# PolyU-IOR/HPR-LP-C

Hardware: AMD Instinct MI355X
Metric: HPR iterations/sec (FP64) (higher is better)
Workload: dtype f64

## Files before the change

### hpr-lp-c_amd/csrc/abi.cpp

```cpp
#include <algorithm>
#include <cmath>
#include <cstdlib>
#include <cstring>
#include <memory>
#include <mutex>
#include <iomanip>
#include <iostream>

#include "hprlp_amd.h"
#include "env.h"
#include "dist.h"
#include "presolve.h"
#include "reorder.h"
#include "solver.h"
#include "version.h"

using namespace hprlp;

struct hprlp_solver {
    Solver s;
    Comm *comm = nullptr;
    Comm *xcomm = nullptr;
    bool sharded = false;
    ~hprlp_solver() {}
// ... 1169 lines not shown
    auto one = [](const char *name, const DeviceMatrix &M) {
        const TiledDev &t = M.view.tiled;
        std::string d = std::string(name) + ": ";
        if (!t.valid) {
            d += "stream kernel (k_spmv_fused, " + std::to_string(M.view.nblk) + " row blocks, " + std::to_string(M.view.nlong) + " split rows)";
            d += no_tiled_note(M.outcome.why);
            return d;
        }
        d += t.n_pieces > 0 ? "tiled, piece form (k_tiled_part + k_tiled_finish, " + std::to_string(t.n_pieces) + " pieces)"
             : t.rem_cap == kPbRemCap ? "tiled, all-remainder form (k_pb_fused, grid " + std::to_string(t.grid) + ")"
                                      : "tiled, fused (k_tiled_fused, grid " + std::to_string(t.grid) + ")";
        d += ", " + std::to_string(t.nsb) + " super-blocks, " + std::to_string(M.tiled.n_steps) + " steps";
        if (t.R != kTileRows || t.T != kTileCols) d += " (" + std::to_string(t.R) + " rows, tiles of " + std::to_string(t.T) + " columns)";
        const double all = static_cast<double>(M.tiled.dense_entries) + static_cast<double>(M.tiled.n_rem);
        if (all > 0) d += ", " + std::to_string(static_cast<int>(100.0 * M.tiled.dense_entries / all + 0.5)) + " % of the entries in staged tiles";
        if (t.f_rk) d += ", source-side run tables";
        if (t.f_work) d += ", pre-pass work list of " + std::to_string(t.n_work) + " workgroups for " + std::to_string(t.n_groups) + " source groups";
        if (t.side_nblk > 0) d += ", long rows aside (" + std::to_string(t.side_nblk) + " blocks through the stream kernel)";
        return d;
    };
    std::string d = one("A", s.A) + "; " + one("A^T", s.AT);
    if (s.use_small && !s.comm) d += "; normal iterations in the single-workgroup kernel (k_small_iterations)";
    if (!s.perm_r.empty()) d += "; locality ordering applied at set-up";
    if (!s.env_at_setup.empty()) d += "; switches: " + s.env_at_setup;
    if (!s.env_ignored_at_setup.empty()) d += "; ignored without HPRLP_TEST_HOOKS=1: " + s.env_ignored_at_setup;
    std::snprintf(buf, static_cast<size_t>(cap), "%s", d.c_str());
    return static_cast<int>(d.size());
    GUARD_END(-1)
}

extern "C" int hprlp_form_select(const hprlp_form_facts *facts, const hprlp_form_hooks *hooks, hprlp_form_decision *out) {
// ... 12 lines not shown
extern "C" int hprlp_solver_form_facts(hprlp_solver *h, int which, hprlp_form_facts out[2]) {
    GUARD_BEGIN
    if (!h || !out || which < 0 || which > 1) throw std::runtime_error("null solver / buffer, or no such matrix");
    h->s.finish_tiling();
    const DeviceMatrix &M = which ? h->s.AT : h->s.A;
    out[0] = M.facts;
    out[1] = M.facts_pb;
    return M.passes;
    GUARD_END(-1)
}

extern "C" int hprlp_tiled_host_check(int m, int n, const int *rowptr, const int *col, int R, int T, double min_dense, long out[6]) {
    try {
        if (m <= 0 || n <= 0 || !rowptr || !col || !out) throw std::runtime_error("bad arguments");
        tiled_host_check(m, n, rowptr, col, R, T, min_dense, out);
        return 0;
    } catch (const std::exception &e) {
        set_last_error(e.what());
        return -1;
    }
}

extern "C" int hprlp_env_switches(char *buf, int cap) {
    int count = 0;
    const EnvEntry *t = env_table(&count);
    std::string d;
    for (int i = 0; i < count; ++i) d += std::string(t[i].name) + "\t" + (t[i].kind == EnvKind::Integrator ? "integrator" : "hook") + "\t" + t[i].what + "\n";
    if (buf && cap > 0) std::snprintf(buf, static_cast<size_t>(cap), "%s", d.c_str());
    return static_cast<int>(d.size());
}
// ... 68 lines not shown
```

### hpr-lp-c_amd/csrc/env.cpp

```cpp
#include "env.h"

#include <cstdlib>
#include <cstring>
#include <stdexcept>

namespace hprlp {

static const EnvEntry kTable[] = {
    {"HPRLP_TEST_HOOKS", EnvKind::Integrator, "1: honour the test hooks below (tests/conftest.py and the tools/ scripts set it)"},
    {"HPRLP_TIMING", EnvKind::Integrator, "wall time of the set-up and solve phases on stderr"},
    {"HPRLP_NO_GRAPH", EnvKind::Integrator, "launch normal iterations eagerly instead of replaying hipGraphs (fall-back)"},
    {"HPRLP_NO_TILED", EnvKind::Integrator, "never build the column-tiled matrix copies: stream kernel everywhere (fall-back)"},
    {"HPRLP_NO_REORDER", EnvKind::Integrator, "no set-up time locality ordering of a large matrix"},
    {"HPRLP_NO_ALLOC_CACHE", EnvKind::Integrator, "do not keep freed device blocks for the next solver of the process"},
    {"HPRLP_DIST_TRANSPORT", EnvKind::Integrator, "shm: hprlp_dist_unique_id names a shared-memory segment (host-staged group of processes on one node) instead of RCCL ids"},
    {"HPRLP_NO_WARM_MODEL", EnvKind::Integrator, "the model constructors do NOT start the HIP runtime / device context / code objects (for a process that forks workers after building its models: a HIP context does not survive fork); the first solve pays for them as in the reference"},
    {"HPRLP_DIST_EXCHANGE", EnvKind::Hook, "sparse | allgather: force the multi-GPU exchange form (same value on every rank)"},
    {"HPRLP_NO_OVERLAP", EnvKind::Integrator, "multi-GPU: shards unsplit, exchange in line on the solver stream"},
    {"HPRLP_DIST_TIMEOUT_S", EnvKind::Integrator, "seconds a rank of the shared-memory transport waits for its peers before it fails (default 120)"},
    {"HPRLP_BATCH_CHUNK", EnvKind::Hook, "solve_batched with 64 or more problems: chunk width of the panels (default 64; narrower chunks map one chunk to each XCD -- measured slower, profiles/r03_tiled_decomposition.md section 6b)"},
    {"HPRLP_BATCH_GRID", EnvKind::Hook, "solve_batched: cap on the row blocks of the normal half-step kernels (read at every call; a small cap makes every workgroup's row loop wrap)"},
    {"HPRLP_BATCH_LAMBDA", EnvKind::Hook, "solve_batched: the batch's lambda_max from the caller (strtod; hand it over as a C99 hex float to keep every bit) instead of 1.01 x the power iteration's estimate (read at every call)"},
    {"HPRLP_COPY_PAUSE_US", EnvKind::Hook, "piece size and pause of the threaded copies of set-up (64 MB, 100 us)"},
    {"HPRLP_COPY_PIECE_MB", EnvKind::Hook, "piece size and pause of the threaded copies of set-up (64 MB, 100 us)"},
    {"HPRLP_DEVICE_TRANSPOSE_MIN", EnvKind::Hook, "build Aᵀ on the host / nonzero threshold of the device transpose (default 4 M)"},
    {"HPRLP_DIST_SELFTEST_FAIL", EnvKind::Hook, "tests only: the set-up self-test of the neighbour exchange reports a failure once (exercises the fall-back to the all-gather)"},
    {"HPRLP_DTON_MAX", EnvKind::Hook, "presolve: cap of the doubleton stage"},
    {"HPRLP_DTON_TRACE", EnvKind::Hook, "presolve: trace the doubleton stage on stderr"},
    {"HPRLP_GEN_FAR", EnvKind::Hook, "benchmark generator: share of a row's entries that fall anywhere (default 0.05)"},
    {"HPRLP_HOST_POWER_START", EnvKind::Hook, "power iteration's start vector made on the host also above 1e6 rows (default there: on the device)"},
    {"HPRLP_HOST_TILING", EnvKind::Hook, "build the tiled copies with the host builder (background threads, default min(16, cores)) instead of on the device"},
    {"HPRLP_HOST_TRANSPOSE", EnvKind::Hook, "build Aᵀ on the host / nonzero threshold of the device transpose (default 4 M)"},
    {"HPRLP_NO_BOUND_CODES", EnvKind::Hook, "the x-half always reads l[j] and u[j], the y-half AL[i] and AU[i] (default: one code byte per column / row says which of them is not a constant; an equality row reads one value)"},
    {"HPRLP_NO_FAR_PUSH", EnvKind::Hook, "always run the remainder pre-pass (k_far_products) instead of the hand-off from the producing half-step's epilogue"},
    {"HPRLP_NO_FAR_WORK", EnvKind::Hook, "the remainder pre-pass with one workgroup per source group also where one group holds several times the mean (default: a work list cuts heavy groups into chunks, tiled.h f_work)"},
    {"HPRLP_NO_PB_LONG_ROWS", EnvKind::Hook, "a matrix kept off the tiled forms for its long rows keeps the stream kernel also where its columns are not popular (default: all-remainder form, Solver::pb_fallback_wanted)"},
    {"HPRLP_NO_FUSED_NORMS", EnvKind::Hook, "the Ruiz row norms by their own passes instead of as a by-product of the preceding scaling pass (same bits)"},
    {"HPRLP_NO_LONG_SIDE", EnvKind::Hook, "a matrix with rows over 1024 entries keeps the stream kernel instead of being tiled with those rows kept aside"},
    {"HPRLP_NO_PB_FALLBACK", EnvKind::Hook, "unstructured large matrices keep the stream kernel instead of the tiled form without dense-tile requirement"},
    {"HPRLP_NO_PB_KERNEL", EnvKind::Hook, "run an all-remainder copy through k_tiled_fused's remainder steps instead of k_pb_fused (A/B)"},
    {"HPRLP_NO_REM2", EnvKind::Hook, "tiled build: no second remainder level"},
    {"HPRLP_NO_SETUP_OVERLAP", EnvKind::Hook, "set-up of a large model in line: no helper threads / copy streams for the value upload, the row blocks, A^T's row pointers and the model vectors (same bits either way)"},
    {"HPRLP_NO_SLAB_CUTS", EnvKind::Hook, "dense rows of a large matrix are not cut at the XCD eighths of the gathered vector (stream kernel)"},
    {"HPRLP_NO_SMALL", EnvKind::Hook, "do not use the single-workgroup kernel for Netlib-scale LPs"},
    {"HPRLP_NO_SMALL_POWER", EnvKind::Hook, "Netlib-scale LPs: power iteration by the regular kernels with the host test every 10th iteration (default: one launch of the single-workgroup kernel)"},
    {"HPRLP_NO_TILED_CR", EnvKind::Hook, "Curtis-Reid passes through the stream kernel also for matrices with a tiled copy (default: tiled kernel on a second value array of -log|a|)"},
    {"HPRLP_NT", EnvKind::Hook, "force default / nontemporal loads of the matrix in the stream kernel"},
    {"HPRLP_OVERLAP_COMM_FIRST", EnvKind::Hook, "tests only: with the in-process rank group, use RCCL's launch order (exchange enqueued before the local SpMV)"},
    {"HPRLP_PB_MIN_COLS", EnvKind::Hook, "gathered-vector length from which an unstructured matrix takes the all-remainder form (default 800 k columns, the crossover measured with k_pb_fused)"},
// ... 64 lines not shown
```

### hpr-lp-c_amd/csrc/kernels.h

```cpp
#pragma once

#include <hip/hip_runtime.h>

#include "tiled.h"

namespace hprlp {

constexpr int kWave = 64;
constexpr int kWavesPerBlock = 4;
constexpr int kThreads = kWave * kWavesPerBlock;
constexpr int kStreamW = 512;
constexpr int kStreamRows = 64;
constexpr int kLongRow = 64;
constexpr int kSplitRow = 4096;
constexpr int kNumScalars = 32;

enum Slot : int {
    S_CX = 0,
    S_YOBJ_Y = 1,
    S_XZ = 2,
    S_RD2 = 3,
    S_RP2 = 4,
    S_ADX_DY = 5,
    S_DY2 = 6,
// ... 47 lines not shown
};

struct Ctrl {
    double sigma, lam_sigma, inv_lam_sigma, inv_sigma;
    int kx, ky;
    int pad0, pad1;
};

struct FarPush {
    const int *gptr = nullptr;
    const double *val = nullptr;
    const int *pos = nullptr;
    const uint16_t *lcol = nullptr;
    double *P = nullptr;
    const int *rptr = nullptr, *rk = nullptr, *rp = nullptr;
};

struct XHalfArgs {
    const double *y_full;
    double *x, *x_hat;
    const double *l, *u, *c, *last_x;
    double *x_bar, *z_bar, *x_temp;
    Ctrl *ctrl;
    double *partials;
    int stride;
    FarPush push;
    bool far_ready = false;
    const unsigned char *lu_code = nullptr;
    int x_mode = 0;
};
// ... 17 lines not shown
void launch_row_codes(int m, const double *AL, const double *AU, unsigned char *code, hipStream_t s);

struct FinalizeItem {
    const double *partials;
    int count;
    int slot;
    int max = 0;
};
struct FinalizeArgs {
    FinalizeItem item[8];
    int n;
};

bool launch_x_half(const CsrDev &AT, const XHalfArgs &a, bool check, hipStream_t s);
bool launch_y_half(const CsrDev &A, const YHalfArgs &a, bool check, hipStream_t s);
FarPush far_push_of(const CsrDev &consumer);
void launch_x_half_base(const CsrDev &AT_remote, const XHalfArgs &a, const double *base, hipStream_t s);
void launch_y_half_base(const CsrDev &A_remote, const YHalfArgs &a, const double *base, hipStream_t s);

void launch_resid_d(const CsrDev &AT, const double *ybar_full, const double *c, const double *z_bar,
                    const double *col_norm, double *partials, hipStream_t s);
void launch_resid_p(const CsrDev &A, const double *xbar_full, const double *xtemp_full, const double *AL,
                    const double *AU, const double *row_norm, const double *y_temp, bool with_gap,
                    double *partials, int stride, hipStream_t s);
void launch_gap(const CsrDev &A, const double *xtemp_full, const double *y_temp, double *partials, hipStream_t s);
bool launch_spmv_push(const CsrDev &M, const double *v_full, double *out, const FarPush &push, hipStream_t s);
void launch_spmv_plain(const CsrDev &M, const double *v_full, double *out, const double *q, bool with_dots,
                       double *partials, int stride, hipStream_t s, bool far_ready = false);

void launch_finalize(const FinalizeArgs &f, double *scalars, hipStream_t s);

// ... 115 lines not shown
```

### hpr-lp-c_amd/csrc/kernels.hip

```cpp
#include "kernels.h"

#include <algorithm>
#include <vector>
#include <cmath>
#include <type_traits>

namespace hprlp {

__device__ __forceinline__ double wave_sum(double v) {
#pragma unroll
    for (int off = 32; off > 0; off >>= 1) v += __shfl_xor(v, off, kWave);
    return v;
}

__device__ __forceinline__ double wave_max(double v) {
#pragma unroll
    for (int off = 32; off > 0; off >>= 1) v = fmax(v, __shfl_xor(v, off, kWave));
    return v;
}

template <int NACC, int NW, int NMAX = 0>
__device__ __forceinline__ void block_store_partials_in(double (&acc)[NACC], double *partials, int stride, double (*red)[NACC > 0 ? NACC : 1]) {
    const int wave = threadIdx.x >> 6, lane = threadIdx.x & 63;
#pragma unroll
// ... 580 lines not shown
        for (int u = 0; u < U; ++u)
            if (k + u * NT < pe) f.P[ps[u]] = prd[u];
    }
}

__device__ __forceinline__ int run_position(const int *tab_k, const int *tab_p, int nr, int k) {
    int lo = 0, hi = nr - 1;
    while (lo < hi) {
        const int mid = (lo + hi + 1) >> 1;
        if (tab_k[mid] <= k) lo = mid;
        else hi = mid - 1;
    }
    return tab_p[lo] + (k - tab_k[lo]);
}

__device__ __forceinline__ void push_products_runs(const FarPush &f, const double *vals, int *tab, int g, int pb, int pe, int tid) {
    constexpr int NT = kTileThreads, U = 4;
    if (pb >= pe) return;
    const int r0 = f.rptr[g], nr = f.rptr[g + 1] - r0;
    int *tab_k = tab, *tab_p = tab + kPbRunTabCap;
    double a4[U];
    uint16_t c4[U];
    auto load_batch = [&](int k0) {
#pragma unroll
        for (int u = 0; u < U; ++u) {
            const int z = min(k0 + u * NT, pe - 1);
            a4[u] = __builtin_nontemporal_load(f.val + z);
            c4[u] = __builtin_nontemporal_load(f.lcol + z);
        }
    };
    int k = pb + tid;
    load_batch(k);
    for (int i = tid; i < nr; i += NT) {
        tab_k[i] = f.rk[r0 + i];
        tab_p[i] = f.rp[r0 + i];
// ... 6 lines not shown
        double prd[U];
        int pc[U];
#pragma unroll
        for (int u = 0; u < U; ++u) {
            prd[u] = a4[u] * vals[c4[u]];
            pc[u] = ps[u];
        }
        const int kn = k + U * NT;
        if (kn < pe) load_batch(kn);
#pragma unroll
        for (int u = 0; u < U; ++u)
            if (k + u * NT < pe) f.P[pc[u]] = prd[u];
        if (kn < pe) {
#pragma unroll
            for (int u = 0; u < U; ++u) ps[u] = run_position(tab_k, tab_p, nr, min(kn + u * NT, pe - 1));
        }
    }
}

template <class Epi, bool REP, bool PUSH = false, bool NARROW = false>
__global__ void __launch_bounds__(kTileThreads, 4) k_tiled_fused(CsrDev A, Epi epi) {
    static_assert(Epi::NV == 1, "the tiled kernel stages one gathered vector");
    constexpr int NT = kTileThreads, RMAX = kTileRows, T = kTileCols;
    constexpr int NACC = Epi::NACC;
    __shared__ double acc[RMAX];
    __shared__ __attribute__((aligned(16))) double ytile[T];
    const TiledDev &t = A.tiled;
    const int tid = threadIdx.x;
    const int R = t.R;
    const int per = t.per, slots = gridDim.x / 8;
// ... 2 lines not shown
#pragma unroll
    for (int i = 0; i < (NACC > 0 ? NACC : 1); ++i) racc[i] = 0.0;
    epi.begin();
    int wg_round = 0;
    const bool wg_stamp = t.wgtimes && tid == 0 && (t.wg_filter == 0 || (PUSH && NACC == 0));
    if (wg_stamp) t.wgtimes[blockIdx.x * 8] = wall_clock64();
    for (int q = slot; q < per; q += slots) {
        const int sb = (blockIdx.x % 8) * per + q;
        if (sb >= t.nsb) break;
        const double *__restrict__ vec = epi.gv[0];
        lds_barrier();
        const int ncols = A.cols;
        for (int i = tid; i < R; i += NT) acc[i] = 0.0;
        const int s0 = t.sb_ptr[sb], smid = t.sb_mid[sb], s1 = t.sb_ptr[sb + 1];
        if (s0 < smid) tiled_sweep<HPRLP_SWEEP_ED, HPRLP_SWEEP_TD, REP, false, LogTerm<Epi>::value, NARROW ? kTileColsNarrow : kTileCols>(t, s0, smid - s0, t.steps[s0].rot, smid - s0, vec, ncols, acc, ytile, tid);
        remainder_steps<kTileRemK>(t, smid, s1, acc, ytile, ytile + kTileRemCap, tid);
        lds_barrier();
        const int r0 = sb * R;
        const int nr = min(R, A.rows - r0);
        int pb = 0, pe = 0;
        if constexpr (PUSH) {
            pb = epi.push.gptr[sb];
            pe = epi.push.gptr[sb + 1];
        }
        epilogue_rows<Epi, PUSH>(epi, acc, racc, r0, nr, tid);
        if constexpr (PUSH) {
            lds_barrier();
            push_products(epi.push, acc, pb, pe, tid);
        }
        if (wg_stamp && ++wg_round <= 5) t.wgtimes[blockIdx.x * 8 + wg_round] = wall_clock64();
    }
    if (wg_stamp) {
        t.wgtimes[blockIdx.x * 8 + 7] = wall_clock64();
        const unsigned hw = __builtin_amdgcn_s_getreg((31 << 11) | 4), xcc = __builtin_amdgcn_s_getreg((31 << 11) | 20);
        t.wgtimes[blockIdx.x * 8 + 6] = (static_cast<unsigned long long>(xcc & 0xfu) << 32) | hw;
    }
    if constexpr (NACC > 0) {
        __syncthreads();
        block_store_partials_in<NACC, kTileThreads / kWave, MaxAccs<Epi>::value>(racc, epi.partials, epi.stride, reinterpret_cast<double(*)[NACC]>(ytile));
    }
}

template <class Epi, bool PUSH = false>
// ... 256 lines not shown
        const int kn = k + U * kFarThreads;
        if (kn < e) load_batch(kn);
#pragma unroll
        for (int u = 0; u < U; ++u)
            if (k + u * kFarThreads < e) t.P[pc[u]] = pr[u];
        if (kn < e) {
#pragma unroll
            for (int u = 0; u < U; ++u) ps[u] = run_position(tab_k, tab_p, nr, min(kn + u * kFarThreads, e - 1));
        }
    }
}

template <bool LOGTERM>
static void launch_far_products(const TiledDev &t, const double *vec, int ncols, hipStream_t s) {
    const dim3 grid(((t.f_work ? t.n_work : t.n_groups) + 7) / 8 * 8);
    if (t.f_rk && t.G <= kPbRowsMax) hipLaunchKernelGGL(k_far_products_runs<LOGTERM>, grid, dim3(kFarThreads), 0, s, t, vec, ncols);
    else hipLaunchKernelGGL(k_far_products<LOGTERM>, grid, dim3(kFarThreads), 0, s, t, vec, ncols);
}


template <bool CHECK, bool STREAMED = false>
struct XEpi {
    static constexpr int NV = 1;
    static constexpr int NACC = CHECK ? 3 : 0;
    const double *gv[1];
    double *x, *x_hat;
    const double *l, *u, *c, *last_x;
    double *x_bar, *z_bar, *x_temp;
    Ctrl *ctrl;
    double *partials;
    int stride;
// ... 424 lines not shown
    }
    if constexpr (Publishes<Epi>::value) {
        if (e.push.gptr) {
            if (narrow) hipLaunchKernelGGL((k_tiled_fused<Epi, false, true, true>), dim3(M.tiled.grid), dim3(kTileThreads), 0, s, M, e);
            else if (M.tiled.repeats) hipLaunchKernelGGL((k_tiled_fused<Epi, true, true>), dim3(M.tiled.grid), dim3(kTileThreads), 0, s, M, e);
            else hipLaunchKernelGGL((k_tiled_fused<Epi, false, true>), dim3(M.tiled.grid), dim3(kTileThreads), 0, s, M, e);
            return true;
        }
    }
    if (narrow) hipLaunchKernelGGL((k_tiled_fused<Epi, false, false, true>), dim3(M.tiled.grid), dim3(kTileThreads), 0, s, M, e);
    else if (M.tiled.repeats) hipLaunchKernelGGL((k_tiled_fused<Epi, true>), dim3(M.tiled.grid), dim3(kTileThreads), 0, s, M, e);
    else hipLaunchKernelGGL((k_tiled_fused<Epi, false>), dim3(M.tiled.grid), dim3(kTileThreads), 0, s, M, e);
    return false;
}

FarPush far_push_of(const CsrDev &consumer) {
    FarPush f;
    if (consumer.tiled.valid && consumer.tiled.n_groups > 0) {
        f.gptr = consumer.tiled.f_gptr;
        f.val = consumer.tiled.f_val;
        f.pos = consumer.tiled.f_pos;
        f.lcol = consumer.tiled.f_lcol;
        f.P = consumer.tiled.P;
        if (consumer.tiled.f_rk) {
            f.rptr = consumer.tiled.f_rptr;
            f.rk = consumer.tiled.f_rk;
            f.rp = consumer.tiled.f_rp;
        }
    }
    return f;
}

bool launch_x_half(const CsrDev &AT, const XHalfArgs &a, bool check, hipStream_t s) {
    if (check) {
        XEpi<true> e{{a.y_full}, a.x, a.x_hat, a.l, a.u, a.c, a.last_x, a.x_bar, a.z_bar, a.x_temp, a.ctrl, a.partials, a.stride, 0, 0, 0, a.push, a.lu_code};
        return launch_fused(AT, e, s, a.far_ready);
    }
    if (AT.tiled.valid) {
        XEpi<false, true> e{{a.y_full}, a.x, a.x_hat, a.l, a.u, a.c, a.last_x, nullptr, nullptr, nullptr, a.ctrl, nullptr, 0, 0, 0, 0, a.push, a.lu_code, a.x_mode};
// ... 1006 lines not shown
```

### hpr-lp-c_amd/csrc/solver.cpp

```cpp
#include "solver.h"
#include "env.h"

#include <algorithm>
#include <cmath>
#include <cstdio>
#include <cstdlib>
#include <cstring>
#include <functional>
#include <iomanip>
#include <iostream>
#include <limits>
#include <thread>

#include "dist.h"
#include "reorder.h"

namespace hprlp {

constexpr int kMaxGraphIters = 64;
constexpr int kDeviceStartRows = 1000000;
constexpr int kPowerBlockKey = -10;

struct RowCuts {
    std::vector<int> rows;
// ... 1297 lines not shown
    HIP_CHECK(hipMemsetAsync(gsm.p, 0, sizeof(double) * m_pad, stream));
    HIP_CHECK(hipMemsetAsync(gsn.p, 0, sizeof(double) * n_pad, stream));
    HIP_CHECK(hipStreamSynchronize(stream));
    power_time = time_since(t0);
    return lambda;
}

void Solver::set_sigma_lambda(double sigma_, double lambda_, bool reset_k) {
    sigma = sigma_;
    lambda_max = lambda_;
    launch_set_ctrl(ctrl.p, sigma, lambda_max, reset_k ? 1 : 0, stream);
}

void Solver::read_hooks() {
    hook_no_far_push = env_get("HPRLP_NO_FAR_PUSH") && env_get("HPRLP_NO_FAR_PUSH")[0] == '1';
    hook_no_bound_codes = env_get("HPRLP_NO_BOUND_CODES") != nullptr;
    hook_store_x = env_get("HPRLP_STORE_X") != nullptr;
}

void Solver::refresh_bound_codes() {
    if (hook_no_bound_codes) return;
    if (n_loc > 0) {
        if (lu_code.n != static_cast<size_t>(n_loc)) lu_code.alloc(static_cast<size_t>(n_loc));
        launch_bound_codes(n_loc, l.p, u.p, lu_code.p, stream);
    }
    if (m_loc > 0) {
        if (row_code.n != static_cast<size_t>(m_loc)) row_code.alloc(static_cast<size_t>(m_loc));
        launch_row_codes(m_loc, AL.p, AU.p, row_code.p, stream);
    }
}
// ... 53 lines not shown
    finish_tiling();
    HIP_CHECK(hipStreamSynchronize(stream));
    ensure_comm_stream();
    ovAT.reset(new SplitShard);
    split_shard(AT, row_off, row_off + m_loc, ovAT.get(), stream);
    ovA.reset(new SplitShard);
    split_shard(A, col_off, col_off + n_loc, ovA.get(), stream);
    HIP_CHECK(hipDeviceSynchronize());
    overlap_ready = true;
}

FarPush Solver::push_into(const DeviceMatrix &consumer, const DeviceMatrix &producer) const {
    const TiledDev &pt = producer.view.tiled;
    if (hook_no_far_push || comm || !pt.valid || pt.n_pieces > 0) return FarPush{};
    if (consumer.view.tiled.valid && consumer.view.tiled.G != pt.R) return FarPush{};
    return far_push_of(consumer.view);
}

int Solver::x_mode_of(int i, int count) const {
    if (hook_store_x || overlap_enabled || !AT.view.tiled.valid) return 0;
    return (i > 0 ? kXRebuild : 0) | (i + 1 < count ? kXNoStore : 0);
}

void Solver::launch_normal_pair(bool more_follow, hipEvent_t *ev, int x_mode) {
    XHalfArgs xa{gy.p, x.p, x_hat, l.p, u.p, c.p, last_x.p, nullptr, nullptr, nullptr, ctrl.p, nullptr, 0};
    xa.lu_code = lu_code.p;
    xa.x_mode = x_mode;
    YHalfArgs ya{gxh.p, y, AL.p, AU.p, last_y.p, nullptr, nullptr, nullptr, ctrl.p, nullptr, 0};
    ya.row_code = row_code.p;
    if (ev) HIP_CHECK(hipEventRecord(ev[0], stream));
    if (!overlap_enabled) {
// ... 542 lines not shown
```

### hpr-lp-c_amd/csrc/solver.h

```cpp
#pragma once

#include <string>
#include <vector>

#include <functional>
#include <future>
#include <map>
#include <memory>

#include "common.h"
#include "env.h"
#include "dist.h"
#include "kernels.h"
#include "hpr_rules.h"
#include "form_select.h"

namespace hprlp {

HPRLP_batched_results solve_batched_impl(const LP_info_cpu *model, int batch_size, const HPRLP_FLOAT *C, const HPRLP_FLOAT *AL,
                                         const HPRLP_FLOAT *AU, const HPRLP_FLOAT *l, const HPRLP_FLOAT *u,
                                         const HPRLP_FLOAT *obj_constants, const HPRLP_parameters *param, const Detection *det,
                                         std::vector<Certificate> *certs, const HPRLP_FLOAT *X0 = nullptr,
                                         const HPRLP_FLOAT *Y0 = nullptr);
HPRLP_batched_results make_batched_error(const char *status, int m, int n, int B);
// ... 145 lines not shown
    void collect_solution(HPRLP_results *out);
    double reduce_sum_sq(const double *v, int n_local);
    void verify_exchange();
    void gather(double *gbuf, bool is_m) { gather_on(gbuf, is_m, stream); }
    void gather_on(double *gbuf, bool is_m, hipStream_t s);

    struct SplitShard {
        DeviceMatrix loc, rem;
        DBuf<double> part;
    };
    std::unique_ptr<SplitShard> ovA, ovAT;
    hipStream_t comm_stream = nullptr;
    hipEvent_t ev_ready = nullptr, ev_done_x = nullptr, ev_done_y = nullptr;
    std::string env_at_setup, env_ignored_at_setup;
    bool hook_no_far_push = false, hook_no_bound_codes = false, hook_store_x = false;
    void read_hooks();
    bool overlap_enabled = false, overlap_ready = false, y_exchange_pending = false;
    bool overlap_spmv_first = false;
    void prepare_overlap();
    void ensure_comm_stream();
    void allreduce_scalars();
    void finish_tiling();

    void launch_normal_pair(bool more_follow = false, hipEvent_t *ev = nullptr, int x_mode = 0);
    int x_mode_of(int i, int count) const;

   private:
    void alloc_work();
    hipGraphExec_t graph_for(int len);
};
// ... 3 lines not shown
```

### hpr-lp-c_amd/csrc/tiled.cpp

```cpp
#include "tiled.h"
#include "env.h"

#include <algorithm>
#include <cstdlib>
#include <cstring>
#include <string>
#include <thread>
#include <type_traits>

namespace hprlp {

namespace {

struct Local {
    std::vector<int> sb_steps, sb_mid;
    std::vector<TileStep> steps;
    std::vector<char> step_is_rem;
    std::vector<uint32_t> tidx;
    std::vector<int> tperm, rcol, rperm;
    std::vector<uint16_t> rrow;
    long dense = 0, pad = 0;
};

void build_range(int rows, int cols, const int *rp, const int *ci, int sb0, int sb1, Local *L, int R, int T, int rem_cap) {
// ... 266 lines not shown
                if (row_of(k) != sb * R + rrow[e]) throw std::runtime_error("tiled check: a remainder entry in the wrong super-block / row");
            }
        }
    }
    for (long k = 0; k < nnz; ++k)
        if (!seen[k]) throw std::runtime_error("tiled check: an entry is missing");
    if (most_run > kTileLayers * ((static_cast<long>(R) * kTileChunk + kTileStepCap - 1) / kTileStepCap + 1)) throw std::runtime_error("tiled check: too many steps for one tile");
    out[0] = static_cast<long>(h.n_tile);
    out[1] = static_cast<long>(h.n_rem);
    out[2] = static_cast<long>(h.steps.size());
    out[3] = pads;
    out[4] = most_run;
    out[5] = static_cast<long>(1e6 * static_cast<double>(h.dense_entries) / static_cast<double>(nnz));
}

void DeviceTiled::upload(const TiledHost &h, int R, int T, int rem_cap) {
    n_tile = static_cast<long>(h.n_tile);
    n_rem = static_cast<long>(h.n_rem);
    n_steps = static_cast<int>(h.steps.size());
    const int nsb = static_cast<int>(h.sb_mid.size());
    sb_ptr.alloc(h.sb_ptr.size()); sb_ptr.upload(h.sb_ptr.data(), h.sb_ptr.size());
    sb_mid.alloc(h.sb_mid.size()); sb_mid.upload(h.sb_mid.data(), h.sb_mid.size());
    steps.alloc(h.steps.size()); steps.upload(h.steps.data(), h.steps.size());
    tidx.alloc_zero(h.n_tile + 8);
    tperm.alloc(h.n_tile + 8);
    tval.alloc_zero(h.n_tile + 8);
    rcol.alloc_zero(h.n_rem + 8);
    rperm.alloc(h.n_rem + 8);
    rrow.alloc_zero(h.n_rem + 8);
    size_t to = 0, ro = 0;
// ... 77 lines not shown
```

### hpr-lp-c_amd/csrc/tiled.h

```cpp
#pragma once

#include <hip/hip_runtime.h>

#include <cstdint>
#include <vector>

#include "common.h"

namespace hprlp {

constexpr int kTileThreads = 512;
constexpr int kTileRows = 8192;
constexpr int kTileCols = 2048;
constexpr int kTileColsNarrow = 1024;
constexpr int kTileChunk = 4;
constexpr int kTileStepCap = kTileThreads * kTileChunk;
constexpr int kTileRemK = 4;
constexpr int kTileRemCap = (kTileThreads - 4) * kTileRemK;
constexpr int kTileRemRun = 16;
#ifndef HPRLP_PB_REM_K
#define HPRLP_PB_REM_K 8
#endif
constexpr int kPbRemK = HPRLP_PB_REM_K;
constexpr int kPbRemCap = kTileThreads * kPbRemK;
constexpr int kPbRowsMax = 4096;
constexpr int kPbRunTabCap = 3072;
constexpr int kTileMaxRow = 1024;
constexpr int kTileDenseMin = 256;
static_assert(kTileRemCap % kTileRemK == 0 && kTileRemCap + (kTileThreads / 64) * 3 / 2 <= kTileCols, "tile buffer too small for the remainder scratch");
constexpr int kTileRowBits = 13;
constexpr int kTileRowsMin = 1024;
static_assert((1 << kTileRowBits) == kTileRows && kTileCols <= (1 << (24 - kTileRowBits)) && kTileChunk == 4,
              "entry codes are 24 bits: 13 of local row, 11 of local column, four per chunk");
inline uint32_t tile_code(int lcol, int row) { return (static_cast<uint32_t>(lcol) << kTileRowBits) | static_cast<uint32_t>(row); }

struct PackLayout {
    int n1 = 0, n2 = 0, n3 = 0, n4 = 0;
    int u3 = 0, u2 = 0, r1 = 0, c2 = 0;
    __host__ __device__ void set(int a1, int a2, int a3, int a4) {
        n1 = a1; n2 = a2; n3 = a3; n4 = a4;
        u3 = n1 < n3 ? n1 : n3;
// ... 78 lines not shown
    const int *sb_mid = nullptr;
    const TileStep *steps = nullptr;
    const double *tval = nullptr;
    const uint32_t *tidx3 = nullptr;
    double *P = nullptr;
    const uint32_t *rq = nullptr;
    int n_groups = 0;
    const int *f_gptr = nullptr;
    const double *f_val = nullptr;
    const int *f_pos = nullptr;
    const uint16_t *f_lcol = nullptr;
    const int *f_rptr = nullptr;
    const int *f_rk = nullptr;
    const int *f_rp = nullptr;
    int f_maxruns = 0;
    const int4 *f_work = nullptr;
    int n_work = 0;
};

struct TiledHost {
    std::vector<int> sb_ptr, sb_mid;
    std::vector<TileStep> steps;
    struct Piece {
        std::vector<uint32_t> tidx;
        std::vector<int> tperm;
        std::vector<int> rcol, rperm;
        std::vector<uint16_t> rrow;
    };
    std::vector<Piece> pieces;
    size_t n_tile = 0, n_rem = 0;
    long dense_entries = 0;
    long padding = 0;
};

bool build_tiled(int rows, int cols, const int *rowptr, const int *col, TiledHost *out, int min_rows,
                 double min_dense_fraction, int R = kTileRows, int T = kTileCols, int rem_cap = kTileRemCap);

void tiled_host_check(int rows, int cols, const int *rp, const int *ci, int R, int T, double min_dense, long out[6]);

void compact_without_rows(long nnz, int rows, const int *rp_dev, const int *rp_c_dev, const int *col_dev, int *col_c, int *map_c, hipStream_t s);

struct DeviceTiled {
    DBuf<int> sb_ptr, sb_mid, tperm, rperm, rcol;
    DBuf<TileStep> steps;
    DBuf<uint32_t> tidx;
    DBuf<uint32_t> tidx3;
    DBuf<uint16_t> rrow;
    DBuf<double> tval;
    DBuf<double> P, f_val;
    DBuf<uint32_t> rq;
    DBuf<int> f_gptr, f_pos, f_perm;
    DBuf<int> f_rptr, f_rk, f_rp;
    DBuf<int4> f_work;
// ... 33 lines not shown
```

### hpr-lp-c_amd/csrc/tiled_build.hip

```cpp
#include <algorithm>
#include <functional>
#include <cstdlib>
#include <hipcub/hipcub.hpp>

#include <vector>

#include "common.h"
#include "env.h"
#include "kernels.h"
#include "tiled.h"

namespace hprlp {

namespace {

constexpr int K = kTileChunk;
constexpr int kRowBits = kTileRowBits;

__device__ __forceinline__ int row_of_entry(const int *__restrict__ rowptr, int rows, int k) {
    int lo = 0, hi = rows;
    while (hi - lo > 1) {
        const int mid = lo + ((hi - lo) >> 1);
        if (rowptr[mid] <= k) lo = mid;
        else hi = mid;
// ... 789 lines not shown
                if (e <= b) continue;
                const long parts = (e - b + cap - 1) / cap, per = (e - b + parts - 1) / parts;
                for (long q = b; q < e; q += per) wl.push_back(make_int4(g, static_cast<int>(q), static_cast<int>(std::min(e, q + per)), 0));
            }
            f_work.alloc(wl.size());
            f_work.upload(wl.data(), wl.size());
            view.f_work = f_work.p;
            view.n_work = static_cast<int>(wl.size());
            if (env_get("HPRLP_TIMING"))
                std::fprintf(stderr, "[timing]   pre-pass work list: %d workgroups for %d source groups (heaviest group %d entries, chunks of at most %ld)\n",
                             view.n_work, ngroups, heaviest, cap);
        }
    }
    view.f_rptr = view.f_rk = view.f_rp = nullptr;
    view.f_maxruns = 0;
    if (view.rem_cap == kPbRemCap) {
        DBuf<int> flag(static_cast<size_t>(n)), excl(static_cast<size_t>(n));
        hipLaunchKernelGGL(k_far_run_flags, dim3(grid_for(n)), dim3(kThreads), 0, s, n, kout.p, f_pos.p, flag.p);
        size_t bytes = 0;
        HIP_CHECK(hipcub::DeviceScan::ExclusiveSum(nullptr, bytes, flag.p, excl.p, n, s));
        {
            DBuf<char> tmp(bytes + 16);
            HIP_CHECK(hipcub::DeviceScan::ExclusiveSum(tmp.p, bytes, flag.p, excl.p, n, s));
            HIP_CHECK(hipStreamSynchronize(s));
        }
        int last_excl = 0, last_flag = 0;
        HIP_CHECK(hipMemcpy(&last_excl, excl.p + (n - 1), sizeof(int), hipMemcpyDeviceToHost));
        HIP_CHECK(hipMemcpy(&last_flag, flag.p + (n - 1), sizeof(int), hipMemcpyDeviceToHost));
        const int nruns = last_excl + last_flag;
        f_rk.alloc(static_cast<size_t>(nruns) + 8);
        f_rp.alloc(static_cast<size_t>(nruns) + 8);
        f_rptr.alloc(static_cast<size_t>(ngroups) + 1);
        DBuf<int> mx;
        mx.alloc_zero(1);
        hipLaunchKernelGGL(k_far_run_fill, dim3(grid_for(n)), dim3(kThreads), 0, s, n, flag.p, excl.p, f_pos.p, f_rk.p, f_rp.p);
        hipLaunchKernelGGL(k_far_rptr, dim3(grid_for(ngroups + 1)), dim3(kThreads), 0, s, ngroups, n, nruns, f_gptr.p, excl.p, f_rptr.p, mx.p);
        int h_mx = 0;
        HIP_CHECK(hipMemcpyAsync(&h_mx, mx.p, sizeof(int), hipMemcpyDeviceToHost, s));
        HIP_CHECK(hipStreamSynchronize(s));
        if (h_mx > 0 && h_mx <= kPbRunTabCap && static_cast<long>(n) >= 48L * nruns) {
            view.f_rptr = f_rptr.p;
            view.f_rk = f_rk.p;
            view.f_rp = f_rp.p;
            view.f_maxruns = h_mx;
        }
        if (env_get("HPRLP_TIMING"))
            std::fprintf(stderr, "[timing]   source-side run tables: %d runs of %d entries (%.1f per run), most in one group %d%s\n", nruns, n,
                         static_cast<double>(n) / std::max(nruns, 1), h_mx, view.f_rk ? "" : " -- not used (too many for the producers' LDS table)");
    }
    rcol.release(); rrow.release(); rperm.release();
    view.P = P.p;
    view.rq = rq.p;
    view.n_groups = ngroups;
    view.f_gptr = f_gptr.p;
    view.f_val = f_val.p;
    view.f_pos = f_pos.p;
    view.f_lcol = f_lcol.p;
}

// ... 166 lines not shown
```

### include/hprlp_amd.h

```cpp
#ifndef HPRLP_AMD_H
#define HPRLP_AMD_H

#include "HPRLP.h"

#ifdef __cplusplus
extern "C" {
#endif

typedef struct hprlp_solver hprlp_solver;

typedef struct hprlp_trace_row {
    int iter, restart_flag;
    double err_Rp, err_Rd, primal_obj, dual_obj, gap, kkt, sigma, current_gap, lambda_max;
} hprlp_trace_row;

const char *hprlp_last_error(void);
const char *hprlp_backend(void);
int hprlp_warmup(int device);
int hprlp_warmup_seconds(double out[4]);

void hprlp_release_device_cache(void);
int hprlp_alloc_cache_selftest(void);

hprlp_solver *hprlp_solver_create(const LP_info_cpu *model, const HPRLP_parameters *param);
// ... 111 lines not shown
                                                   hprlp_local_group *group);

typedef struct hprlp_presolve hprlp_presolve;
hprlp_presolve *hprlp_presolve_run(const LP_info_cpu *model);
const LP_info_cpu *hprlp_presolve_reduced(const hprlp_presolve *p);
int hprlp_presolve_stats(const hprlp_presolve *p, int out[16]);
int hprlp_presolve_postsolve(const hprlp_presolve *p, const double *xr, const double *yr, const double *zr, double *x,
                             double *y, double *z);
int hprlp_presolve_forward(const hprlp_presolve *p, const double *x, const double *y, double *xr, double *yr);
void hprlp_presolve_free(hprlp_presolve *p);
int hprlp_original_kkt(const LP_info_cpu *model, const double *x, const double *y, const double *z, double out[5]);

int hprlp_locality_ordering(int m, int n, const int *rowptr, const int *col, int *row_new2old, int *col_new2old, double out[6]);
int hprlp_row_block_plan(int m, int n, const int *rowptr, const int *col, int with_cuts, long out[6]);
int hprlp_tiled_host_check(int m, int n, const int *rowptr, const int *col, int R, int T, double min_dense, long out[6]);

typedef struct hprlp_form_built {
    long ok;
    long n_pieces, dense_entries, n_rem;
    double rem_top_share;
} hprlp_form_built;
typedef struct hprlp_form_facts {
    long rows, cols, nnz, longest_row;
    double long_row_share;
    double line_density;
    double xcd_gather_bytes;
    long sb_rows, slots;
    double min_dense_override;
    long sharded;
    long heaviest_block;
// ... 35 lines not shown
```

Baseline: 748.7.

## Use run tables and early-issued loads in the tiled fused kernel's hand-off

Extends the source-side run tables, previously built only for the all-remainder form, to the tiled fused kernel's far-product hand-off, so it can compute write positions from a small LDS run table instead of reading f_pos per entry. It also issues the first trip of hand-off loads (values, local columns, run entries) before the epilogue so their latency overlaps epilogue work. The cost is more registers held across the epilogue, a reused LDS scratch area, and an extra table build for all matrices. A hook picks the mode, and a host reference builder is added for testing.

Measured after the change: 748.5 (median of 3 runs). About the same (-0.0%).

```diff
diff --git a/hpr-lp-c_amd/csrc/abi.cpp b/hpr-lp-c_amd/csrc/abi.cpp
--- a/hpr-lp-c_amd/csrc/abi.cpp
+++ b/hpr-lp-c_amd/csrc/abi.cpp
@@ -1207,7 +1207,9 @@
         if (t.R != kTileRows || t.T != kTileCols) d += " (" + std::to_string(t.R) + " rows, tiles of " + std::to_string(t.T) + " columns)";
         const double all = static_cast<double>(M.tiled.dense_entries) + static_cast<double>(M.tiled.n_rem);
         if (all > 0) d += ", " + std::to_string(static_cast<int>(100.0 * M.tiled.dense_entries / all + 0.5)) + " % of the entries in staged tiles";
-        if (t.f_rk) d += ", source-side run tables";
+        if (t.f_rk) d += t.rem_cap == kPbRemCap ? ", source-side run tables" : ", hand-off positions from run tables";
+        else if (t.n_groups > 0 && t.rem_cap != kPbRemCap && t.f_maxruns > kTileRunTabCap)
+            d += ", hand-off positions kept in f_pos (" + std::to_string(t.f_maxruns) + " runs in one source group)";
         if (t.f_work) d += ", pre-pass work list of " + std::to_string(t.n_work) + " workgroups for " + std::to_string(t.n_groups) + " source groups";
         if (t.side_nblk > 0) d += ", long rows aside (" + std::to_string(t.side_nblk) + " blocks through the stream kernel)";
         return d;
@@ -1250,6 +1252,28 @@
     try {
         if (m <= 0 || n <= 0 || !rowptr || !col || !out) throw std::runtime_error("bad arguments");
         tiled_host_check(m, n, rowptr, col, R, T, min_dense, out);
+        return 0;
+    } catch (const std::exception &e) {
+        set_last_error(e.what());
+        return -1;
+    }
+}
+
+extern "C" int hprlp_far_tables_host(int m, int n, const int *rowptr, const int *col, int R, int T, double min_dense, int G, long cap,
+                                     int *f_gptr, int *f_pos, int *f_rptr, int *f_rk, int *f_rp, long out[3]) {
+    try {
+        if (m <= 0 || n <= 0 || !rowptr || !col || !out || !f_gptr || !f_pos || !f_rptr || !f_rk || !f_rp) throw std::runtime_error("bad arguments");
+        FarTablesHost t;
+        far_tables_host(m, n, rowptr, col, R, T, min_dense, G, &t);
+        if (static_cast<long>(t.f_pos.size()) > cap) throw std::runtime_error("far tables: buffers too small");
+        std::copy(t.f_gptr.begin(), t.f_gptr.end(), f_gptr);
+        std::copy(t.f_pos.begin(), t.f_pos.end(), f_pos);
+        std::copy(t.f_rptr.begin(), t.f_rptr.end(), f_rptr);
+        std::copy(t.f_rk.begin(), t.f_rk.end(), f_rk);
+        std::copy(t.f_rp.begin(), t.f_rp.end(), f_rp);
+        out[0] = static_cast<long>(t.f_pos.size());
+        out[1] = static_cast<long>(t.f_rk.size());
+        out[2] = t.maxruns;
         return 0;
     } catch (const std::exception &e) {
         set_last_error(e.what());
diff --git a/hpr-lp-c_amd/csrc/env.cpp b/hpr-lp-c_amd/csrc/env.cpp
--- a/hpr-lp-c_amd/csrc/env.cpp
+++ b/hpr-lp-c_amd/csrc/env.cpp
@@ -33,6 +33,7 @@
     {"HPRLP_HOST_TRANSPOSE", EnvKind::Hook, "build Aᵀ on the host / nonzero threshold of the device transpose (default 4 M)"},
     {"HPRLP_NO_BOUND_CODES", EnvKind::Hook, "the x-half always reads l[j] and u[j], the y-half AL[i] and AU[i] (default: one code byte per column / row says which of them is not a constant; an equality row reads one value)"},
     {"HPRLP_NO_FAR_PUSH", EnvKind::Hook, "always run the remainder pre-pass (k_far_products) instead of the hand-off from the producing half-step's epilogue"},
+    {"HPRLP_HANDOFF_MODE", EnvKind::Hook, "hand-off of k_tiled_fused: 0 = positions from f_pos and the whole hand-off behind the epilogue (the form before the run tables; tests, same-box A/B), 1 = run tables only, 2 = first trip before the epilogue only, 3 = both (default)"},
     {"HPRLP_NO_FAR_WORK", EnvKind::Hook, "the remainder pre-pass with one workgroup per source group also where one group holds several times the mean (default: a work list cuts heavy groups into chunks, tiled.h f_work)"},
     {"HPRLP_NO_PB_LONG_ROWS", EnvKind::Hook, "a matrix kept off the tiled forms for its long rows keeps the stream kernel also where its columns are not popular (default: all-remainder form, Solver::pb_fallback_wanted)"},
     {"HPRLP_NO_FUSED_NORMS", EnvKind::Hook, "the Ruiz row norms by their own passes instead of as a by-product of the preceding scaling pass (same bits)"},
diff --git a/hpr-lp-c_amd/csrc/kernels.h b/hpr-lp-c_amd/csrc/kernels.h
--- a/hpr-lp-c_amd/csrc/kernels.h
+++ b/hpr-lp-c_amd/csrc/kernels.h
@@ -85,6 +85,7 @@
     const uint16_t *lcol = nullptr;
     double *P = nullptr;
     const int *rptr = nullptr, *rk = nullptr, *rp = nullptr;
+    int early = 0;
 };
 
 struct XHalfArgs {
@@ -132,7 +133,7 @@
 
 bool launch_x_half(const CsrDev &AT, const XHalfArgs &a, bool check, hipStream_t s);
 bool launch_y_half(const CsrDev &A, const YHalfArgs &a, bool check, hipStream_t s);
-FarPush far_push_of(const CsrDev &consumer);
+FarPush far_push_of(const CsrDev &consumer, bool producer_pb = false, int mode = 3);
 void launch_x_half_base(const CsrDev &AT_remote, const XHalfArgs &a, const double *base, hipStream_t s);
 void launch_y_half_base(const CsrDev &A_remote, const YHalfArgs &a, const double *base, hipStream_t s);
 
diff --git a/hpr-lp-c_amd/csrc/kernels.hip b/hpr-lp-c_amd/csrc/kernels.hip
--- a/hpr-lp-c_amd/csrc/kernels.hip
+++ b/hpr-lp-c_amd/csrc/kernels.hip
@@ -618,11 +618,12 @@
     return tab_p[lo] + (k - tab_k[lo]);
 }
 
+template <int CAP = kPbRunTabCap>
 __device__ __forceinline__ void push_products_runs(const FarPush &f, const double *vals, int *tab, int g, int pb, int pe, int tid) {
     constexpr int NT = kTileThreads, U = 4;
     if (pb >= pe) return;
     const int r0 = f.rptr[g], nr = f.rptr[g + 1] - r0;
-    int *tab_k = tab, *tab_p = tab + kPbRunTabCap;
+    int *tab_k = tab, *tab_p = tab + CAP;
     double a4[U];
     uint16_t c4[U];
     auto load_batch = [&](int k0) {
@@ -659,6 +660,86 @@
         if (kn < pe) {
 #pragma unroll
             for (int u = 0; u < U; ++u) ps[u] = run_position(tab_k, tab_p, nr, min(kn + u * NT, pe - 1));
+        }
+    }
+}
+
+struct PushHead {
+    double a4[4];
+    uint16_t c4[4];
+    int q[8];
+};
+
+template <bool RUNS>
+__device__ __forceinline__ void push_early_begin(const FarPush &f, PushHead &h, int r0, int nr, int pb, int pe, int tid) {
+    constexpr int NT = kTileThreads, U = 4;
+    static_assert(U * NT >= kTileRunTabCap, "a lane holds four runs of the table");
+    if (pb >= pe) return;
+    if constexpr (RUNS) {
+#pragma unroll
+        for (int u = 0; u < U; ++u) {
+            const int i = r0 + min(tid + u * NT, nr - 1);
+            h.q[u] = f.rk[i];
+            h.q[U + u] = f.rp[i];
+        }
+    }
+#pragma unroll
+    for (int u = 0; u < U; ++u) {
+        const int z = min(pb + tid + u * NT, pe - 1);
+        h.a4[u] = __builtin_nontemporal_load(f.val + z);
+        if constexpr (!RUNS) h.q[u] = __builtin_nontemporal_load(f.pos + z);
+        h.c4[u] = __builtin_nontemporal_load(f.lcol + z);
+    }
+}
+
+template <bool RUNS>
+__device__ __forceinline__ void push_early_finish(const FarPush &f, const double *vals, PushHead &h, int *tab, int nr, int pb, int pe, int tid) {
+    constexpr int NT = kTileThreads, U = 4;
+    int *tab_k = tab, *tab_p = tab + kTileRunTabCap;
+    if constexpr (RUNS) {
+        if (pb < pe) {
+#pragma unroll
+            for (int u = 0; u < U; ++u) {
+                const int i = tid + u * NT;
+                if (i < nr) {
+                    tab_k[i] = h.q[u];
+                    tab_p[i] = h.q[U + u];
+                }
+            }
+        }
+    }
+    lds_barrier();
+    if (pb >= pe) return;
+    int k = pb + tid;
+    int ps[U];
+#pragma unroll
+    for (int u = 0; u < U; ++u) ps[u] = RUNS ? run_position(tab_k, tab_p, nr, min(k + u * NT, pe - 1)) : h.q[u];
+    for (; k < pe; k += U * NT) {
+        double prd[U];
+        int pc[U];
+#pragma unroll
+        for (int u = 0; u < U; ++u) {
+            prd[u] = h.a4[u] * vals[h.c4[u]];
+            pc[u] = ps[u];
+        }
+        const int kn = k + U * NT;
+        if (kn < pe) {
+#pragma unroll
+            for (int u = 0; u < U; ++u) {
+                const int z = min(kn + u * NT, pe - 1);
+                h.a4[u] = __builtin_nontemporal_load(f.val + z);
+                if constexpr (!RUNS) ps[u] = __builtin_nontemporal_load(f.pos + z);
+                h.c4[u] = __builtin_nontemporal_load(f.lcol + z);
+            }
+        }
+#pragma unroll
+        for (int u = 0; u < U; ++u)
+            if (k + u * NT < pe) f.P[pc[u]] = prd[u];
+        if constexpr (RUNS) {
+            if (kn < pe) {
+#pragma unroll
+                for (int u = 0; u < U; ++u) ps[u] = run_position(tab_k, tab_p, nr, min(kn + u * NT, pe - 1));
+            }
         }
     }
 }
@@ -691,19 +772,40 @@
         for (int i = tid; i < R; i += NT) acc[i] = 0.0;
         const int s0 = t.sb_ptr[sb], smid = t.sb_mid[sb], s1 = t.sb_ptr[sb + 1];
         if (s0 < smid) tiled_sweep<HPRLP_SWEEP_ED, HPRLP_SWEEP_TD, REP, false, LogTerm<Epi>::value, NARROW ? kTileColsNarrow : kTileCols>(t, s0, smid - s0, t.steps[s0].rot, smid - s0, vec, ncols, acc, ytile, tid);
+        int pb = 0, pe = 0, run0 = 0, nruns = 0;
+        bool runs = false, early = false;
+        if constexpr (PUSH) {
+            pb = epi.push.gptr[sb];
+            pe = epi.push.gptr[sb + 1];
+            runs = epi.push.rk != nullptr;
+            early = epi.push.early != 0;
+            if (runs) {
+                run0 = epi.push.rptr[sb];
+                nruns = epi.push.rptr[sb + 1] - run0;
+            }
+        }
         remainder_steps<kTileRemK>(t, smid, s1, acc, ytile, ytile + kTileRemCap, tid);
         lds_barrier();
         const int r0 = sb * R;
         const int nr = min(R, A.rows - r0);
-        int pb = 0, pe = 0;
+        PushHead head;
         if constexpr (PUSH) {
-            pb = epi.push.gptr[sb];
-            pe = epi.push.gptr[sb + 1];
+            if (early) {
+                if (runs) push_early_begin<true>(epi.push, head, run0, nruns, pb, pe, tid);
+                else push_early_begin<false>(epi.push, head, 0, 0, pb, pe, tid);
+            }
         }
         epilogue_rows<Epi, PUSH>(epi, acc, racc, r0, nr, tid);
         if constexpr (PUSH) {
-            lds_barrier();
-            push_products(epi.push, acc, pb, pe, tid);
+            int *tab = reinterpret_cast<int *>(ytile);
+            if (early) {
+                if (runs) push_early_finish<true>(epi.push, acc, head, tab, nruns, pb, pe, tid);
+                else push_early_finish<false>(epi.push, acc, head, tab, 0, pb, pe, tid);
+            } else {
+                lds_barrier();
+                if (runs) push_products_runs<kTileRunTabCap>(epi.push, acc, tab, sb, pb, pe, tid);
+                else push_products(epi.push, acc, pb, pe, tid);
+            }
         }
         if (wg_stamp && ++wg_round <= 5) t.wgtimes[blockIdx.x * 8 + wg_round] = wall_clock64();
     }
@@ -990,7 +1092,7 @@
 template <bool LOGTERM>
 static void launch_far_products(const TiledDev &t, const double *vec, int ncols, hipStream_t s) {
     const dim3 grid(((t.f_work ? t.n_work : t.n_groups) + 7) / 8 * 8);
-    if (t.f_rk && t.G <= kPbRowsMax) hipLaunchKernelGGL(k_far_products_runs<LOGTERM>, grid, dim3(kFarThreads), 0, s, t, vec, ncols);
+    if (t.f_rk && t.f_runs_pb && t.G <= kPbRowsMax) hipLaunchKernelGGL(k_far_products_runs<LOGTERM>, grid, dim3(kFarThreads), 0, s, t, vec, ncols);
     else hipLaunchKernelGGL(k_far_products<LOGTERM>, grid, dim3(kFarThreads), 0, s, t, vec, ncols);
 }
 
@@ -1445,7 +1547,7 @@
     return false;
 }
 
-FarPush far_push_of(const CsrDev &consumer) {
+FarPush far_push_of(const CsrDev &consumer, bool producer_pb, int mode) {
     FarPush f;
     if (consumer.tiled.valid && consumer.tiled.n_groups > 0) {
         f.gptr = consumer.tiled.f_gptr;
@@ -1453,7 +1555,8 @@
         f.pos = consumer.tiled.f_pos;
         f.lcol = consumer.tiled.f_lcol;
         f.P = consumer.tiled.P;
-        if (consumer.tiled.f_rk) {
+        f.early = (mode & 2) ? 1 : 0;
+        if (consumer.tiled.f_rk && (producer_pb ? consumer.tiled.f_runs_pb : (consumer.tiled.f_runs_tiled && (mode & 1)))) {
             f.rptr = consumer.tiled.f_rptr;
             f.rk = consumer.tiled.f_rk;
             f.rp = consumer.tiled.f_rp;
diff --git a/hpr-lp-c_amd/csrc/solver.cpp b/hpr-lp-c_amd/csrc/solver.cpp
--- a/hpr-lp-c_amd/csrc/solver.cpp
+++ b/hpr-lp-c_amd/csrc/solver.cpp
@@ -1335,6 +1335,7 @@
 
 void Solver::read_hooks() {
     hook_no_far_push = env_get("HPRLP_NO_FAR_PUSH") && env_get("HPRLP_NO_FAR_PUSH")[0] == '1';
+    if (const char *hm = env_get("HPRLP_HANDOFF_MODE"); hm && hm[0] >= '0' && hm[0] <= '3') hook_handoff_mode = hm[0] - '0';
     hook_no_bound_codes = env_get("HPRLP_NO_BOUND_CODES") != nullptr;
     hook_store_x = env_get("HPRLP_STORE_X") != nullptr;
 }
@@ -1418,7 +1419,7 @@
     const TiledDev &pt = producer.view.tiled;
     if (hook_no_far_push || comm || !pt.valid || pt.n_pieces > 0) return FarPush{};
     if (consumer.view.tiled.valid && consumer.view.tiled.G != pt.R) return FarPush{};
-    return far_push_of(consumer.view);
+    return far_push_of(consumer.view, pt.rem_cap == kPbRemCap, hook_handoff_mode);
 }
 
 int Solver::x_mode_of(int i, int count) const {
diff --git a/hpr-lp-c_amd/csrc/solver.h b/hpr-lp-c_amd/csrc/solver.h
--- a/hpr-lp-c_amd/csrc/solver.h
+++ b/hpr-lp-c_amd/csrc/solver.h
@@ -183,6 +183,7 @@
     hipEvent_t ev_ready = nullptr, ev_done_x = nullptr, ev_done_y = nullptr;
     std::string env_at_setup, env_ignored_at_setup;
     bool hook_no_far_push = false, hook_no_bound_codes = false, hook_store_x = false;
+    int hook_handoff_mode = 3;
     void read_hooks();
     bool overlap_enabled = false, overlap_ready = false, y_exchange_pending = false;
     bool overlap_spmv_first = false;
diff --git a/hpr-lp-c_amd/csrc/tiled.cpp b/hpr-lp-c_amd/csrc/tiled.cpp
--- a/hpr-lp-c_amd/csrc/tiled.cpp
+++ b/hpr-lp-c_amd/csrc/tiled.cpp
@@ -304,6 +304,43 @@
     out[5] = static_cast<long>(1e6 * static_cast<double>(h.dense_entries) / static_cast<double>(nnz));
 }
 
+void far_tables_host(int rows, int cols, const int *rp, const int *ci, int R, int T, double min_dense, int G, FarTablesHost *out) {
+    TiledHost h;
+    if (G < 64 || G > kFarGroup) throw std::runtime_error("remainder lists: unsupported source-group size");
+    if (!build_tiled(rows, cols, rp, ci, &h, 1, min_dense, R, T, kTileRemCap)) throw std::runtime_error("far tables: the build declined the pattern");
+    std::vector<int> rcol;
+    for (const TiledHost::Piece &pc : h.pieces) rcol.insert(rcol.end(), pc.rcol.begin(), pc.rcol.end());
+    const int n = static_cast<int>(rcol.size()), nsb = static_cast<int>(h.sb_mid.size()), ngroups = (cols + G - 1) / G;
+    std::vector<int> sb_of(static_cast<size_t>(n), -1);
+    for (int sb = 0; sb < nsb; ++sb)
+        for (int s = h.sb_mid[sb]; s < h.sb_ptr[sb + 1]; ++s)
+            for (int e = h.steps[s].e_begin; e < h.steps[s].e_end; ++e) sb_of[e] = sb;
+    std::vector<int> e_of_p(static_cast<size_t>(n)), p_of_f(static_cast<size_t>(n));
+    for (int e = 0; e < n; ++e) e_of_p[e] = e;
+    std::stable_sort(e_of_p.begin(), e_of_p.end(), [&](int a, int b) { return sb_of[a] != sb_of[b] ? sb_of[a] < sb_of[b] : rcol[a] / G < rcol[b] / G; });
+    for (int p = 0; p < n; ++p) p_of_f[p] = p;
+    std::stable_sort(p_of_f.begin(), p_of_f.end(), [&](int a, int b) { return rcol[e_of_p[a]] / G < rcol[e_of_p[b]] / G; });
+    out->f_pos = p_of_f;
+    out->f_gptr.assign(static_cast<size_t>(ngroups) + 1, n);
+    for (int f = n - 1; f >= 0; --f) out->f_gptr[rcol[e_of_p[p_of_f[f]]] / G] = f;
+    for (int g = ngroups - 1; g >= 0; --g) out->f_gptr[g] = std::min(out->f_gptr[g], out->f_gptr[g + 1]);
+    out->f_rptr.assign(static_cast<size_t>(ngroups) + 1, 0);
+    out->f_rk.clear();
+    out->f_rp.clear();
+    out->maxruns = 0;
+    for (int g = 0; g < ngroups; ++g) {
+        out->f_rptr[g] = static_cast<int>(out->f_rk.size());
+        for (int f = out->f_gptr[g]; f < out->f_gptr[g + 1]; ++f) {
+            if (f == out->f_gptr[g] || out->f_pos[f] != out->f_pos[f - 1] + 1) {
+                out->f_rk.push_back(f);
+                out->f_rp.push_back(out->f_pos[f]);
+            }
+        }
+        out->maxruns = std::max(out->maxruns, static_cast<int>(out->f_rk.size()) - out->f_rptr[g]);
+    }
+    out->f_rptr[ngroups] = static_cast<int>(out->f_rk.size());
+}
+
 void DeviceTiled::upload(const TiledHost &h, int R, int T, int rem_cap) {
     n_tile = static_cast<long>(h.n_tile);
     n_rem = static_cast<long>(h.n_rem);
diff --git a/hpr-lp-c_amd/csrc/tiled.h b/hpr-lp-c_amd/csrc/tiled.h
--- a/hpr-lp-c_amd/csrc/tiled.h
+++ b/hpr-lp-c_amd/csrc/tiled.h
@@ -25,6 +25,7 @@
 constexpr int kPbRemCap = kTileThreads * kPbRemK;
 constexpr int kPbRowsMax = 4096;
 constexpr int kPbRunTabCap = 3072;
+constexpr int kTileRunTabCap = kTileCols / 2;
 constexpr int kTileMaxRow = 1024;
 constexpr int kTileDenseMin = 256;
 static_assert(kTileRemCap % kTileRemK == 0 && kTileRemCap + (kTileThreads / 64) * 3 / 2 <= kTileCols, "tile buffer too small for the remainder scratch");
@@ -133,6 +134,8 @@
     const int *f_rk = nullptr;
     const int *f_rp = nullptr;
     int f_maxruns = 0;
+    bool f_runs_pb = false;
+    bool f_runs_tiled = false;
     const int4 *f_work = nullptr;
     int n_work = 0;
 };
@@ -156,6 +159,12 @@
                  double min_dense_fraction, int R = kTileRows, int T = kTileCols, int rem_cap = kTileRemCap);
 
 void tiled_host_check(int rows, int cols, const int *rp, const int *ci, int R, int T, double min_dense, long out[6]);
+
+struct FarTablesHost {
+    std::vector<int> f_gptr, f_pos, f_rptr, f_rk, f_rp;
+    int maxruns = 0;
+};
+void far_tables_host(int rows, int cols, const int *rp, const int *ci, int R, int T, double min_dense, int G, FarTablesHost *out);
 
 void compact_without_rows(long nnz, int rows, const int *rp_dev, const int *rp_c_dev, const int *col_dev, int *col_c, int *map_c, hipStream_t s);
 
diff --git a/hpr-lp-c_amd/csrc/tiled_build.hip b/hpr-lp-c_amd/csrc/tiled_build.hip
--- a/hpr-lp-c_amd/csrc/tiled_build.hip
+++ b/hpr-lp-c_amd/csrc/tiled_build.hip
@@ -827,7 +827,8 @@
     }
     view.f_rptr = view.f_rk = view.f_rp = nullptr;
     view.f_maxruns = 0;
-    if (view.rem_cap == kPbRemCap) {
+    view.f_runs_pb = view.f_runs_tiled = false;
+    {
         DBuf<int> flag(static_cast<size_t>(n)), excl(static_cast<size_t>(n));
         hipLaunchKernelGGL(k_far_run_flags, dim3(grid_for(n)), dim3(kThreads), 0, s, n, kout.p, f_pos.p, flag.p);
         size_t bytes = 0;
@@ -851,11 +852,15 @@
         int h_mx = 0;
         HIP_CHECK(hipMemcpyAsync(&h_mx, mx.p, sizeof(int), hipMemcpyDeviceToHost, s));
         HIP_CHECK(hipStreamSynchronize(s));
-        if (h_mx > 0 && h_mx <= kPbRunTabCap && static_cast<long>(n) >= 48L * nruns) {
+        view.f_maxruns = h_mx;
+        view.f_runs_pb = view.rem_cap == kPbRemCap && h_mx > 0 && h_mx <= kPbRunTabCap && static_cast<long>(n) >= 48L * nruns;
+        view.f_runs_tiled = h_mx > 0 && h_mx <= kTileRunTabCap && (view.rem_cap != kPbRemCap || view.f_runs_pb);
+        if (view.f_runs_pb || view.f_runs_tiled) {
             view.f_rptr = f_rptr.p;
             view.f_rk = f_rk.p;
             view.f_rp = f_rp.p;
-            view.f_maxruns = h_mx;
+        } else {
+            f_rptr.release(); f_rk.release(); f_rp.release();
         }
         if (env_get("HPRLP_TIMING"))
             std::fprintf(stderr, "[timing]   source-side run tables: %d runs of %d entries (%.1f per run), most in one group %d%s\n", nruns, n,
diff --git a/include/hprlp_amd.h b/include/hprlp_amd.h
--- a/include/hprlp_amd.h
+++ b/include/hprlp_amd.h
@@ -149,6 +149,8 @@
 int hprlp_locality_ordering(int m, int n, const int *rowptr, const int *col, int *row_new2old, int *col_new2old, double out[6]);
 int hprlp_row_block_plan(int m, int n, const int *rowptr, const int *col, int with_cuts, long out[6]);
 int hprlp_tiled_host_check(int m, int n, const int *rowptr, const int *col, int R, int T, double min_dense, long out[6]);
+int hprlp_far_tables_host(int m, int n, const int *rowptr, const int *col, int R, int T, double min_dense, int G, long cap,
+                          int *f_gptr, int *f_pos, int *f_rptr, int *f_rk, int *f_rp, long out[3]);
 
 typedef struct hprlp_form_built {
     long ok;
```
